# Wendison/FCL-taco2

Hardware: AMD Instinct MI355X
Metric: mel-frames/sec (FCL-taco2-S forward, batch=32, 80-mel) (higher is better)
Workload: dtype f32 via bf16x3-split MFMA operands, fp32 accumulate (max-abs 8e-6 on mel vs the reference; FCL_PRECISION=0 = exact fp32 MFMA)

## Files before the change

### fcl-taco2_amd/csrc/decoder_step.hip

```cpp
#include "fcl_common.h"
#include "lstm_epilogue.h"

namespace fcl {


template <int NT>
__device__ __forceinline__ void rowtile_mma(const float* A_l, int lda_l, const float* const (&wrow)[NT], int K, int r16, int kq,
                                            f32x4 (&out)[NT], int rot = 0) {
    f32x4 acc0[NT], acc1[NT];
#pragma unroll
    for (int t = 0; t < NT; ++t) acc0[t] = acc1[t] = (f32x4){0.f, 0.f, 0.f, 0.f};
    const float* ap = A_l + r16 * lda_l + kq * 4;
    const float* wp[NT];
#pragma unroll
    for (int t = 0; t < NT; ++t) wp[t] = wrow[t] + kq * 4;
    const int nfull = K >> 6;
    f32x4 bn[NT][4];
    int cc = nfull > 0 ? rot % nfull : 0;
    if (nfull > 0) {
#pragma unroll
        for (int t = 0; t < NT; ++t)
#pragma unroll
            for (int i = 0; i < 4; ++i) bn[t][i] = *reinterpret_cast<const f32x4*>(wp[t] + (cc << 6) + i * 16);
    }
    for (int c = 0; c < nfull; ++c) {
        const int k = cc << 6;
        const int cn = cc + 1 == nfull ? 0 : cc + 1;
        f32x4 b[NT][4], a[4];
#pragma unroll
        for (int t = 0; t < NT; ++t)
#pragma unroll
            for (int i = 0; i < 4; ++i) b[t][i] = bn[t][i];
        if (c + 1 < nfull) {
#pragma unroll
            for (int t = 0; t < NT; ++t)
#pragma unroll
                for (int i = 0; i < 4; ++i) bn[t][i] = *reinterpret_cast<const f32x4*>(wp[t] + (cn << 6) + i * 16);
        }
        cc = cn;
#pragma unroll
        for (int i = 0; i < 4; ++i) a[i] = *reinterpret_cast<const f32x4*>(ap + k + i * 16);
        __builtin_amdgcn_sched_barrier(0);
#pragma unroll
        for (int i = 0; i < 4; ++i) {
#pragma unroll
            for (int t = 0; t < NT; ++t) {
                acc0[t] = __builtin_amdgcn_mfma_f32_16x16x4f32(a[i][0], b[t][i][0], acc0[t], 0, 0, 0);
                acc1[t] = __builtin_amdgcn_mfma_f32_16x16x4f32(a[i][1], b[t][i][1], acc1[t], 0, 0, 0);
            }
#pragma unroll
            for (int t = 0; t < NT; ++t) {
                acc0[t] = __builtin_amdgcn_mfma_f32_16x16x4f32(a[i][2], b[t][i][2], acc0[t], 0, 0, 0);
                acc1[t] = __builtin_amdgcn_mfma_f32_16x16x4f32(a[i][3], b[t][i][3], acc1[t], 0, 0, 0);
            }
        }
    }
    for (int k = nfull << 6; k < K; k += 16) {
        const bool in = k + kq * 4 < K;
        f32x4 a = *reinterpret_cast<const f32x4*>(in ? ap + k : A_l + r16 * lda_l);
        if (!in) a = (f32x4){0.f, 0.f, 0.f, 0.f};
#pragma unroll
        for (int t = 0; t < NT; ++t) {
            const f32x4 bb = *reinterpret_cast<const f32x4*>(in ? wp[t] + k : wrow[t]);
            acc0[t] = __builtin_amdgcn_mfma_f32_16x16x4f32(a[0], bb[0], acc0[t], 0, 0, 0);
            acc1[t] = __builtin_amdgcn_mfma_f32_16x16x4f32(a[1], bb[1], acc1[t], 0, 0, 0);
            acc0[t] = __builtin_amdgcn_mfma_f32_16x16x4f32(a[2], bb[2], acc0[t], 0, 0, 0);
            acc1[t] = __builtin_amdgcn_mfma_f32_16x16x4f32(a[3], bb[3], acc1[t], 0, 0, 0);
        }
    }
#pragma unroll
    for (int t = 0; t < NT; ++t) out[t] = acc0[t] + acc1[t];
}

__device__ __forceinline__ void load_rowtile(float* dst, int ld_l, const float* src, int ld, int K, int m0, int M) {
    const int per_row = K >> 2;
    for (int i = threadIdx.x; i < 16 * per_row; i += blockDim.x) {
        const int r = i / per_row, c = (i - r * per_row) * 4;
        const int m = min(m0 + r, M - 1);
        *reinterpret_cast<f32x4*>(dst + r * ld_l + c) = *reinterpret_cast<const f32x4*>(src + (size_t)m * ld + c);
    }
}

__device__ __forceinline__ float drop_apply(float v, int mode, const uint8_t* keep, int ldkeep, int m, int n, int N,
                                            float scale, float p, unsigned int seed) {
    if (mode == 1) return keep[(size_t)m * ldkeep + n] ? v * scale : 0.f;
    if (mode == 2) {
        const unsigned int h = hash_u32(((unsigned int)m * (unsigned int)N + (unsigned int)n) ^ seed);
        return ((h >> 8) * (1.0f / 16777216.0f) >= p) ? v * scale : 0.f;
    }
    return v;
}

__device__ __forceinline__ bool feat_prenet_rows(const FeatPrenetArgs& a, int rows, int& Ms_feat, int& Ms_pre) {
    Ms_feat = (a.live && a.t_prev >= 0) ? min(a.M_feat, a.live[a.t_prev]) : a.M_feat;
    Ms_pre = a.live ? min(a.M_pre, a.live[a.t_cur]) : a.M_pre;
    if (a.live && a.w0 && blockIdx.x == 0 && threadIdx.x == 0 && a.live[a.t_cur] > a.M_pre) atomicOr(a.status, (unsigned int)FCL_STATUS_ROWS_CAP);
    if ((int)blockIdx.x * rows >= (a.h1 ? Ms_feat : Ms_pre)) return false;
    return true;
}

__global__ __launch_bounds__(512) void feat_prenet_kernel(const FeatPrenetArgs a) {
    const int M_feat = a.M_feat, M_pre = a.M_pre;
    int Ms_feat, Ms_pre;
    if (!feat_prenet_rows(a, 16, Ms_feat, Ms_pre)) return;
    extern __shared__ __attribute__((aligned(16))) float smem[];
    const int ldU = a.U + 4, ldO = a.O + 4, ldP = a.P + 4;
    float* A1 = smem;
    float* A2 = A1 + 16 * ldU;
    float* A3 = A2 + 16 * ldO;
    const int m0 = blockIdx.x * 16;
    const int lane = threadIdx.x & 63, wave = threadIdx.x >> 6, nwaves = blockDim.x >> 6;
    const int r16 = lane & 15, kq = lane >> 4;
    const int col = lane & 15, rq = lane >> 4;
    const unsigned int sbump = a.seed_dev ? *a.seed_dev * 0x9E3779B9u : 0u;
    const unsigned int seed0 = hash_u32(a.seed0 + sbump), seed1 = hash_u32(a.seed1 + sbump);

    if (a.h1) {
        load_rowtile(A1, ldU, a.h1, a.U, a.U, m0, M_feat);
        __syncthreads();
        for (int tile = wave; tile * 16 < a.O; tile += nwaves) {
            const float* const wr[1] = {a.wf_h + (size_t)min(tile * 16 + r16, a.O - 1) * a.U};
            const int nc = tile * 16 + col, ncc = min(nc, a.O - 1);
            float f0v[4];
            int fo[4];
#pragma unroll
            for (int r = 0; r < 4; ++r) {
                const int mc = min(m0 + rq * 4 + r, M_feat - 1);
                f0v[r] = a.F0[(size_t)mc * a.O + ncc];
                fo[r] = a.frame_off[mc];
            }
            f32x4 accv[1];
            rowtile_mma<1>(A1, ldU, wr, a.U, r16, kq, accv, blockIdx.x);
            const f32x4 acc = accv[0];
#pragma unroll
            for (int r = 0; r < 4; ++r) {
                const int row = rq * 4 + r, m = m0 + row;
                float v = 0.f;
                if (m < Ms_feat && nc < a.O) {
                    v = acc[r] + f0v[r];
                    a.before[(size_t)(fo[r] + a.t_prev) * a.O + nc] = v;
                }
                if (nc < a.O) A2[row * ldO + nc] = (a.out_act && m < Ms_feat) ? act_apply(v, a.out_act) : v;
            }
        }
    } else {
        for (int i = threadIdx.x; i < 16 * ldO; i += blockDim.x) A2[i] = 0.f;
    }
    if (!a.w0 || m0 >= M_pre) return;
    __syncthreads();
    if (a.teacher_in) {
        load_rowtile(A2, ldO, a.teacher_in, a.teacher_ld, a.O, m0, M_pre);
        __syncthreads();
    }
    for (int tile = wave; tile * 16 < a.P; tile += 2 * nwaves) {
        const int tile2 = tile + nwaves;
        const float* const wr[2] = {a.w0 + (size_t)min(tile * 16 + r16, a.P - 1) * a.O, a.w0 + (size_t)min(tile2 * 16 + r16, a.P - 1) * a.O};
        f32x4 accv[2];
        rowtile_mma<2>(A2, ldO, wr, a.O, r16, kq, accv, blockIdx.x);
#pragma unroll
        for (int tt = 0; tt < 2; ++tt) {
            const int nc = (tt ? tile2 : tile) * 16 + col;
            if (nc < a.P) {
                const float bn = a.b0[nc];
#pragma unroll
                for (int r = 0; r < 4; ++r) {
                    const int row = rq * 4 + r, m = m0 + row;
                    float v = fmaxf(accv[tt][r] + bn, 0.f);
                    if (m < M_pre) v = drop_apply(v, a.drop_mode, a.keep0, a.P, m, nc, a.P, a.keep_scale, a.drop_p, seed0);
                    A3[row * ldP + nc] = v;
                }
            }
        }
    }
    __syncthreads();
    for (int tile = wave; tile * 16 < a.P; tile += 2 * nwaves) {
        const int tile2 = tile + nwaves;
        const float* const wr[2] = {a.w1 + (size_t)min(tile * 16 + r16, a.P - 1) * a.P, a.w1 + (size_t)min(tile2 * 16 + r16, a.P - 1) * a.P};
        f32x4 accv[2];
        rowtile_mma<2>(A3, ldP, wr, a.P, r16, kq, accv, blockIdx.x);
#pragma unroll
        for (int tt = 0; tt < 2; ++tt) {
            const int nc = (tt ? tile2 : tile) * 16 + col;
            if (nc < a.P) {
                const float bn = a.b1[nc];
#pragma unroll
                for (int r = 0; r < 4; ++r) {
                    const int m = m0 + rq * 4 + r;
                    if (m >= Ms_pre) continue;
                    float v = fmaxf(accv[tt][r] + bn, 0.f);
                    v = drop_apply(v, a.drop_mode, a.keep1, a.P, m, nc, a.P, a.keep_scale, a.drop_p, seed1);
                    a.pre_out[(size_t)m * a.P + nc] = v;
                    if (a.tap_prenet) a.tap_prenet[(size_t)(a.frame_off[m] + a.t_cur) * a.P + nc] = v;
                }
            }
        }
    }
}

__device__ __forceinline__ void split1(float x, u16& hi, u16& lo) {
    const __bf16 h = (__bf16)x;
    hi = __builtin_bit_cast(u16, h);
    lo = __builtin_bit_cast(u16, (__bf16)(x - (float)h));
}

template <int NT>
__device__ __forceinline__ void rowtile_mma_x3(const u16* Ah, const u16* Al, int ldk, const u16* const (&fhi)[NT], const u16* const (&flo)[NT],
                                               int K, int r16, int kq, f32x4 (&out)[NT]) {
    f32x4 acc[NT];
#pragma unroll
    for (int t = 0; t < NT; ++t) acc[t] = (f32x4){0.f, 0.f, 0.f, 0.f};
    const u16* ah = Ah + r16 * ldk + kq * 8;
    const u16* al = Al + r16 * ldk + kq * 8;
    const int nsteps = (K + 31) >> 5;
    s16x8 bhn[NT], bln[NT];
#pragma unroll
    for (int t = 0; t < NT; ++t) {
        bhn[t] = *reinterpret_cast<const s16x8*>(fhi[t]);
        bln[t] = *reinterpret_cast<const s16x8*>(flo[t]);
    }
    for (int st = 0; st < nsteps; ++st) {
        const int k = st << 5;
        s16x8 bh[NT], bl[NT];
#pragma unroll
        for (int t = 0; t < NT; ++t) { bh[t] = bhn[t]; bl[t] = bln[t]; }
        if (st + 1 < nsteps) {
#pragma unroll
            for (int t = 0; t < NT; ++t) {
                bhn[t] = *reinterpret_cast<const s16x8*>(fhi[t] + (size_t)(st + 1) * 512);
                bln[t] = *reinterpret_cast<const s16x8*>(flo[t] + (size_t)(st + 1) * 512);
            }
        }
        s16x8 a_hi = {0, 0, 0, 0, 0, 0, 0, 0}, a_lo = {0, 0, 0, 0, 0, 0, 0, 0};
        if (k + kq * 8 < K) {
            a_hi = *reinterpret_cast<const s16x8*>(ah + k);
            a_lo = *reinterpret_cast<const s16x8*>(al + k);
        }
        __builtin_amdgcn_sched_barrier(0);
#pragma unroll
        for (int t = 0; t < NT; ++t) acc[t] = __builtin_amdgcn_mfma_f32_16x16x32_bf16(a_lo, bh[t], acc[t], 0, 0, 0);
#pragma unroll
        for (int t = 0; t < NT; ++t) acc[t] = __builtin_amdgcn_mfma_f32_16x16x32_bf16(a_hi, bl[t], acc[t], 0, 0, 0);
#pragma unroll
        for (int t = 0; t < NT; ++t) acc[t] = __builtin_amdgcn_mfma_f32_16x16x32_bf16(a_hi, bh[t], acc[t], 0, 0, 0);
    }
#pragma unroll
    for (int t = 0; t < NT; ++t) out[t] = acc[t];
}

template <int NT, int NS>
struct WFrag {
    s16x8 hi[NT][NS], lo[NT][NS];
    __device__ __forceinline__ void load(const u16* const (&fhi)[NT], const u16* const (&flo)[NT]) {
#pragma unroll
        for (int t = 0; t < NT; ++t)
#pragma unroll
            for (int st = 0; st < NS; ++st) {
                hi[t][st] = *reinterpret_cast<const s16x8*>(fhi[t] + st * 512);
                lo[t][st] = *reinterpret_cast<const s16x8*>(flo[t] + st * 512);
            }
    }
    __device__ __forceinline__ void mma(const u16* Ah, const u16* Al, int ldk, int K, int r16, int kq, f32x4 (&out)[NT]) const {
        f32x4 acc[NT];
#pragma unroll
        for (int t = 0; t < NT; ++t) acc[t] = (f32x4){0.f, 0.f, 0.f, 0.f};
        const u16* ah = Ah + r16 * ldk + kq * 8;
        const u16* al = Al + r16 * ldk + kq * 8;
#pragma unroll
        for (int st = 0; st < NS; ++st) {
            s16x8 a_hi = {0, 0, 0, 0, 0, 0, 0, 0}, a_lo = {0, 0, 0, 0, 0, 0, 0, 0};
            if (st * 32 + kq * 8 < K) {
                a_hi = *reinterpret_cast<const s16x8*>(ah + st * 32);
                a_lo = *reinterpret_cast<const s16x8*>(al + st * 32);
            }
#pragma unroll
            for (int t = 0; t < NT; ++t) acc[t] = __builtin_amdgcn_mfma_f32_16x16x32_bf16(a_lo, hi[t][st], acc[t], 0, 0, 0);
#pragma unroll
            for (int t = 0; t < NT; ++t) acc[t] = __builtin_amdgcn_mfma_f32_16x16x32_bf16(a_hi, lo[t][st], acc[t], 0, 0, 0);
#pragma unroll
            for (int t = 0; t < NT; ++t) acc[t] = __builtin_amdgcn_mfma_f32_16x16x32_bf16(a_hi, hi[t][st], acc[t], 0, 0, 0);
        }
#pragma unroll
        for (int t = 0; t < NT; ++t) out[t] = acc[t];
    }
};

__device__ __forceinline__ void load_rowtile_split(u16* Ah, u16* Al, int ldk, const float* src, int ld, int K, int m0, int M) {
    const int per_row = K >> 2;
    for (int i = threadIdx.x; i < 16 * per_row; i += blockDim.x) {
        const int r = i / per_row, c = (i - r * per_row) * 4;
        const int m = min(m0 + r, M - 1);
        const f32x4 v = *reinterpret_cast<const f32x4*>(src + (size_t)m * ld + c);
        u16 h[4], l[4];
#pragma unroll
        for (int e = 0; e < 4; ++e) split1(v[e], h[e], l[e]);
        *reinterpret_cast<uint2*>(Ah + r * ldk + c) = make_uint2(h[0] | ((unsigned)h[1] << 16), h[2] | ((unsigned)h[3] << 16));
        *reinterpret_cast<uint2*>(Al + r * ldk + c) = make_uint2(l[0] | ((unsigned)l[1] << 16), l[2] | ((unsigned)l[3] << 16));
    }
}

__global__ __launch_bounds__(512) void feat_prenet_x3_kernel(const FeatPrenetArgs a) {
    const int M_feat = a.M_feat, M_pre = a.M_pre;
    const int Ms_feat = (a.live && a.t_prev >= 0) ? min(a.M_feat, a.live[a.t_prev]) : a.M_feat, Ms_pre = a.live ? min(a.M_pre, a.live[a.t_cur]) : a.M_pre;
    if (a.live && a.w0 && blockIdx.x == 0 && threadIdx.x == 0 && a.live[a.t_cur] > a.M_pre) atomicOr(a.status, (unsigned int)FCL_STATUS_ROWS_CAP);
    if ((int)blockIdx.x * (16) >= (a.h1 ? Ms_feat : Ms_pre)) return;
    extern __shared__ __attribute__((aligned(16))) float smem[];
    const int ldU = a.U + 8, ldO = a.O + 8, ldP = a.P + 8;
    u16* A1h = reinterpret_cast<u16*>(smem);
    u16* A1l = A1h + 16 * ldU;
    u16* A2h = A1l + 16 * ldU;
    u16* A2l = A2h + 16 * ldO;
    u16* A3h = A2l + 16 * ldO;
    u16* A3l = A3h + 16 * ldP;
    const int m0 = blockIdx.x * 16;
    const int lane = threadIdx.x & 63, wave = threadIdx.x >> 6, nwaves = blockDim.x >> 6;
    const int r16 = lane & 15, kq = lane >> 4;
    const int col = lane & 15, rq = lane >> 4;
    const unsigned int sbump = a.seed_dev ? *a.seed_dev * 0x9E3779B9u : 0u;
    const unsigned int seed0 = hash_u32(a.seed0 + sbump), seed1 = hash_u32(a.seed1 + sbump);

    const bool has_pre = a.w0 && m0 < M_pre;
    const int ptile = wave, ptile2 = wave + nwaves;
    const int nsU = (a.U + 31) >> 5, nsO = (a.O + 31) >> 5, nsP = (a.P + 31) >> 5, ptmax = ((a.P + 15) >> 4) - 1;
    const size_t lane8 = (size_t)lane * 8;
    auto frag = [&](const u16* base, int tile, int ns) { return base + (size_t)tile * ns * 512 + lane8; };
    float pb0[2] = {0.f, 0.f}, pb1[2] = {0.f, 0.f};
    if (has_pre) {
#pragma unroll
        for (int tt = 0; tt < 2; ++tt) {
            const int nc = min((tt ? ptile2 : ptile) * 16 + col, a.P - 1);
            pb0[tt] = a.b0[nc];
            pb1[tt] = a.b1[nc];
        }
    }
    if (a.h1) {
        f32x4 accv[1];
        load_rowtile_split(A1h, A1l, ldU, a.h1, a.U, a.U, m0, M_feat);
        __syncthreads();
        if (a.dbg_phase == 1) return;
        for (int tile = wave; tile * 16 < a.O; tile += nwaves) {
            const u16* const wh[1] = {frag(a.wf_hi, tile, nsU)};
            const u16* const wl[1] = {frag(a.wf_lo, tile, nsU)};
            const int nc = tile * 16 + col, ncc = min(nc, a.O - 1);
            float f0v[4];
            int fo[4];
#pragma unroll
            for (int r = 0; r < 4; ++r) {
                const int mc = min(m0 + rq * 4 + r, M_feat - 1);
                f0v[r] = a.F0[(size_t)mc * a.O + ncc];
                fo[r] = a.frame_off[mc];
            }
            rowtile_mma_x3<1>(A1h, A1l, ldU, wh, wl, a.U, r16, kq, accv);
#pragma unroll
            for (int r = 0; r < 4; ++r) {
                const int row = rq * 4 + r, m = m0 + row;
                float v = 0.f;
                if (m < Ms_feat && nc < a.O) {
                    v = accv[0][r] + f0v[r];
                    a.before[(size_t)(fo[r] + a.t_prev) * a.O + nc] = v;
                    if (a.before_p) store_p32(a.before_p, (a.O + 31) >> 5, fo[r] + a.t_prev, nc, v);
                }
                if (nc < a.O) split1((a.out_act && m < Ms_feat) ? act_apply(v, a.out_act) : v, A2h[row * ldO + nc], A2l[row * ldO + nc]);
            }
        }
        if (a.before_p && (a.O & 31)) {
            const int padc = 32 - (a.O & 31);
            for (int i = threadIdx.x; i < 16 * padc; i += blockDim.x) {
                const int m = m0 + i / padc;
                if (m < Ms_feat) store_p32(a.before_p, (a.O + 31) >> 5, a.frame_off[m] + a.t_prev, a.O + i % padc, 0.f);
            }
        }
    } else {
        for (int i = threadIdx.x; i < 16 * ldO; i += blockDim.x) { A2h[i] = 0; A2l[i] = 0; }
    }
    if (!has_pre || a.dbg_phase == 2) return;
    lds_barrier();
    if (a.teacher_in) {
        load_rowtile_split(A2h, A2l, ldO, a.teacher_in, a.teacher_ld, a.O, m0, M_pre);
        __syncthreads();
    }
    for (int tile = wave; tile * 16 < a.P; tile += 2 * nwaves) {
        const int tile2 = tile + nwaves;
        const u16* const wh[2] = {frag(a.w0_hi, tile, nsO), frag(a.w0_hi, min(tile2, ptmax), nsO)};
        const u16* const wl[2] = {frag(a.w0_lo, tile, nsO), frag(a.w0_lo, min(tile2, ptmax), nsO)};
        f32x4 accv[2];
        rowtile_mma_x3<2>(A2h, A2l, ldO, wh, wl, a.O, r16, kq, accv);
#pragma unroll
        for (int tt = 0; tt < 2; ++tt) {
            const int nc = (tt ? tile2 : tile) * 16 + col;
            if (nc < a.P) {
                const float bn = tile == ptile ? pb0[tt] : a.b0[nc];
#pragma unroll
                for (int r = 0; r < 4; ++r) {
                    const int row = rq * 4 + r, m = m0 + row;
                    float v = fmaxf(accv[tt][r] + bn, 0.f);
                    if (m < M_pre) v = drop_apply(v, a.drop_mode, a.keep0, a.P, m, nc, a.P, a.keep_scale, a.drop_p, seed0);
                    split1(v, A3h[row * ldP + nc], A3l[row * ldP + nc]);
                }
            }
        }
    }
    lds_barrier();
    if (a.dbg_phase == 3) return;
    for (int tile = wave; tile * 16 < a.P; tile += 2 * nwaves) {
        const int tile2 = tile + nwaves;
        const u16* const wh[2] = {frag(a.w1_hi, tile, nsP), frag(a.w1_hi, min(tile2, ptmax), nsP)};
        const u16* const wl[2] = {frag(a.w1_lo, tile, nsP), frag(a.w1_lo, min(tile2, ptmax), nsP)};
        f32x4 accv[2];
        rowtile_mma_x3<2>(A3h, A3l, ldP, wh, wl, a.P, r16, kq, accv);
#pragma unroll
        for (int tt = 0; tt < 2; ++tt) {
            const int nc = (tt ? tile2 : tile) * 16 + col;
            if (nc < a.P) {
                const float bn = tile == ptile ? pb1[tt] : a.b1[nc];
#pragma unroll
                for (int r = 0; r < 4; ++r) {
                    const int m = m0 + rq * 4 + r;
                    if (m >= Ms_pre) continue;
                    float v = fmaxf(accv[tt][r] + bn, 0.f);
                    v = drop_apply(v, a.drop_mode, a.keep1, a.P, m, nc, a.P, a.keep_scale, a.drop_p, seed1);
                    if (a.pre_out) a.pre_out[(size_t)m * a.P + nc] = v;
                    if (a.pre_out_p) store_p32(a.pre_out_p, (a.P + 31) >> 5, m, nc, v);
                    if (a.tap_prenet) a.tap_prenet[(size_t)(a.frame_off[m] + a.t_cur) * a.P + nc] = v;
                }
            }
        }
    }
}

__device__ __forceinline__ void p32_store4(unsigned short* __restrict__ p, int ld, long long m, int n, uint2 hi, uint2 lo) {
    unsigned short* line = p + ((size_t)m * ld + (n >> 5)) * 64 + (n & 31);
    *reinterpret_cast<uint2*>(line) = hi;
    *reinterpret_cast<uint2*>(line + 32) = lo;
}

template <int NT, int NS_>
__device__ __forceinline__ void mma_t(const WFrag<NT, NS_>& w, const u16* Ah, const u16* Al, int ldk, int r16, int kq, f32x4 (&out)[NT]) {
    f32x4 acc[NT];
#pragma unroll
    for (int t = 0; t < NT; ++t) acc[t] = (f32x4){0.f, 0.f, 0.f, 0.f};
    const u16* ah = Ah + r16 * ldk + kq * 8;
    const u16* al = Al + r16 * ldk + kq * 8;
#pragma unroll
    for (int st = 0; st < NS_; ++st) {
        const s16x8 a_hi = *reinterpret_cast<const s16x8*>(ah + st * 32);
        const s16x8 a_lo = *reinterpret_cast<const s16x8*>(al + st * 32);
#pragma unroll
        for (int t = 0; t < NT; ++t) acc[t] = __builtin_amdgcn_mfma_f32_16x16x32_bf16(w.hi[t][st], a_lo, acc[t], 0, 0, 0);
#pragma unroll
        for (int t = 0; t < NT; ++t) acc[t] = __builtin_amdgcn_mfma_f32_16x16x32_bf16(w.lo[t][st], a_hi, acc[t], 0, 0, 0);
#pragma unroll
        for (int t = 0; t < NT; ++t) acc[t] = __builtin_amdgcn_mfma_f32_16x16x32_bf16(w.hi[t][st], a_hi, acc[t], 0, 0, 0);
    }
#pragma unroll
    for (int t = 0; t < NT; ++t) out[t] = acc[t];
}

template <int DROP, int RT>
__global__ __launch_bounds__(512) void feat_prenet_split_kernel(const FeatPrenetArgs a) {
    constexpr int SU = 8, SO = 3, SP = 8, U = 256, OP = 96, P = 256;
    const int M_feat = a.M_feat, M_pre = a.M_pre;
    const int Ms_feat = (a.live && a.t_prev >= 0) ? min(a.M_feat, a.live[a.t_prev]) : a.M_feat, Ms_pre = a.live ? min(a.M_pre, a.live[a.t_cur]) : a.M_pre;
    const int split = blockIdx.y;
    if (a.live && a.w0 && blockIdx.x == 0 && split == 0 && threadIdx.x == 0 && a.live[a.t_cur] > a.M_pre) atomicOr(a.status, (unsigned int)FCL_STATUS_ROWS_CAP);
    if ((int)blockIdx.x * (16 * RT) >= (a.h1 ? Ms_feat : Ms_pre)) return;
    constexpr int ldU = U + 16, ldO = OP + 16, ldP = P + 16, ROWS = 16 * RT;
    static_assert(ldU == ldP, "the layer-1 operand tile re-uses the h1 tile's LDS");
    extern __shared__ __attribute__((aligned(16))) u16 fp_lds[];
    u16* A1h = fp_lds;
    u16* A1l = A1h + ROWS * ldU;
    u16* A2h = A1l + ROWS * ldU;
    u16* A2l = A2h + ROWS * ldO;
    u16* A3h = A1h;
    u16* A3l = A1l;
    const int O = a.O;
    const int m0 = blockIdx.x * ROWS;
    const int lane = threadIdx.x & 63, wave = __builtin_amdgcn_readfirstlane(threadIdx.x >> 6);
    const int r16 = lane & 15, kq = lane >> 4;
    const int arow = lane & 15, cq = lane >> 4;
    const bool has_feat = a.h1 != nullptr, has_pre = a.w0 != nullptr && m0 < M_pre;
    if (!has_pre && split != 0) return;
    const bool feat_wave = has_feat && wave * 16 < O;
    const size_t lane8 = (size_t)lane * 8;
    auto frag = [&](const u16* base, int tile, int ns) { return base + (size_t)tile * ns * 512 + lane8; };
    const int t0 = wave, t1 = wave + 8;
    const int c1 = split * 16 + wave * 2;

    constexpr int HV = RT * 2;
    f32x4 hreg[HV];
    if (has_feat) {
#pragma unroll
        for (int j = 0; j < HV; ++j) {
            const int i = threadIdx.x + j * 512, r = i >> 6, c = (i & 63) * 4;
            hreg[j] = *reinterpret_cast<const f32x4*>(a.h1 + (size_t)min(m0 + r, M_feat - 1) * U + c);
        }
    }
    asm volatile("s_barrier" ::: "memory");
    WFrag<1, SU> ff;
    WFrag<2, SO> f0;
    WFrag<2, SP> f1;
    const int fnc = wave * 16 + cq * 4;
    f32x4 f0v[RT];
    int fo[RT];
    if (feat_wave) {
        const u16* const wh[1] = {frag(a.wf_hi, wave, SU)};
        const u16* const wl[1] = {frag(a.wf_lo, wave, SU)};
        ff.load(wh, wl);
    }
#pragma unroll
    for (int q = 0; q < RT; ++q) {
        f0v[q] = (f32x4){0.f, 0.f, 0.f, 0.f};
        fo[q] = 0;
        if (feat_wave && fnc < O) {
            const int mc = min(m0 + q * 16 + arow, M_feat - 1);
            f0v[q] = *reinterpret_cast<const f32x4*>(a.F0 + (size_t)mc * O + fnc);
            if (split == 0) fo[q] = a.frame_off[mc];
        }
    }
    unsigned int seed0 = 0, seed1 = 0;
    const unsigned int thr16 = (unsigned int)(a.drop_p * 65536.0f);
    if (DROP == 2) {
        const unsigned int sbump = a.seed_dev ? *a.seed_dev * 0x9E3779B9u : 0u;
        seed0 = hash_u32(a.seed0 + sbump);
        seed1 = hash_u32(a.seed1 + sbump);
    }
    f32x4 pb0[2], pb1[2];
    unsigned int k0[RT][2], k1[RT][2];
#pragma unroll
    for (int tt = 0; tt < 2; ++tt) pb0[tt] = (f32x4){0.f, 0.f, 0.f, 0.f};
    if (has_feat) asm volatile("s_barrier" ::: "memory");
    if (has_pre) {
        const u16* const wh0[2] = {frag(a.w0_hi, t0, SO), frag(a.w0_hi, t1, SO)};
        const u16* const wl0[2] = {frag(a.w0_lo, t0, SO), frag(a.w0_lo, t1, SO)};
        f0.load(wh0, wl0);
#pragma unroll
        for (int tt = 0; tt < 2; ++tt) {
            const int nc = (tt ? t1 : t0) * 16 + cq * 4;
            pb0[tt] = *reinterpret_cast<const f32x4*>(a.b0 + nc);
            if (DROP == 1) {
#pragma unroll
                for (int q = 0; q < RT; ++q) k0[q][tt] = *reinterpret_cast<const unsigned int*>(a.keep0 + (size_t)min(m0 + q * 16 + arow, M_pre - 1) * P + nc);
            }
        }
    }
    for (int i = threadIdx.x; i < ROWS * ldO / 8; i += 512) {
        reinterpret_cast<uint4*>(A2h)[i] = make_uint4(0, 0, 0, 0);
        reinterpret_cast<uint4*>(A2l)[i] = make_uint4(0, 0, 0, 0);
    }
    if (has_feat) {
#pragma unroll
        for (int j = 0; j < HV; ++j) {
            const int i = threadIdx.x + j * 512, r = i >> 6, c = (i & 63) * 4;
            uint2 h, l;
            split4(hreg[j], h, l);
            *reinterpret_cast<uint2*>(A1h + r * ldU + c) = h;
            *reinterpret_cast<uint2*>(A1l + r * ldU + c) = l;
        }
    }
#pragma unroll
    for (int tt = 0; tt < 2; ++tt) pb1[tt] = (f32x4){0.f, 0.f, 0.f, 0.f};
    auto request_l1 = [&]() {
        if (has_pre) {
            const u16* wh1[2];
            const u16* wl1[2];
#pragma unroll
            for (int tt = 0; tt < 2; ++tt) {
                wh1[tt] = frag(a.w1_hi, c1 + tt, SP);
                wl1[tt] = frag(a.w1_lo, c1 + tt, SP);
            }
            f1.load(wh1, wl1);
#pragma unroll
            for (int tt = 0; tt < 2; ++tt) {
                const int nc = (c1 + tt) * 16 + cq * 4;
                pb1[tt] = *reinterpret_cast<const f32x4*>(a.b1 + nc);
                if (DROP == 1) {
#pragma unroll
                    for (int q = 0; q < RT; ++q) k1[q][tt] = *reinterpret_cast<const unsigned int*>(a.keep1 + (size_t)min(m0 + q * 16 + arow, M_pre - 1) * P + nc);
                }
            }
        }
    };
    lds_barrier();
    if (a.dbg_phase == 1) return;
    if (feat_wave) {
#pragma unroll
        for (int q = 0; q < RT; ++q) {
            f32x4 accv[1];
            mma_t<1, SU>(ff, A1h + q * 16 * ldU, A1l + q * 16 * ldU, ldU, r16, kq, accv);
            const int row = q * 16 + arow, m = m0 + row;
            if (fnc < O) {
                f32x4 v = (f32x4){0.f, 0.f, 0.f, 0.f};
                uint2 h, l;
                if (m < Ms_feat) {
                    v = accv[0] + f0v[q];
                    if (split == 0) {
                        const long long fr = (long long)fo[q] + a.t_prev;
                        *reinterpret_cast<f32x4*>(a.before + (size_t)fr * O + fnc) = v;
                        if (a.before_p) {
                            split4(v, h, l);
                            p32_store4(a.before_p, (O + 31) >> 5, fr, fnc, h, l);
                        }
                    }
                    if (a.out_act) {
#pragma unroll
                        for (int r = 0; r < 4; ++r) v[r] = act_apply(v[r], a.out_act);
                    }
                }
                split4(v, h, l);
                *reinterpret_cast<uint2*>(A2h + row * ldO + fnc) = h;
                *reinterpret_cast<uint2*>(A2l + row * ldO + fnc) = l;
            }
        }
    }
    if (has_feat && split == 0 && a.before_p && (O & 31)) {
        const int padc = 32 - (O & 31);
        for (int i = threadIdx.x; i < ROWS * padc; i += 512) {
            const int m = m0 + i / padc;
            if (m < Ms_feat) store_p32(a.before_p, (O + 31) >> 5, a.frame_off[m] + a.t_prev, O + i % padc, 0.f);
        }
    }
    if (!has_pre || a.dbg_phase == 2) return;
    request_l1();
    lds_barrier();
    if (a.teacher_in) {
#pragma unroll
        for (int q = 0; q < RT; ++q) load_rowtile_split(A2h + q * 16 * ldO, A2l + q * 16 * ldO, ldO, a.teacher_in, a.teacher_ld, O, m0 + q * 16, M_pre);
        lds_barrier();
    }
#pragma unroll
    for (int q = 0; q < RT; ++q) {
        f32x4 accv[2];
        mma_t<2, SO>(f0, A2h + q * 16 * ldO, A2l + q * 16 * ldO, ldO, r16, kq, accv);
        const int row = q * 16 + arow, m = m0 + row;
#pragma unroll
        for (int tt = 0; tt < 2; ++tt) {
            const int nc = (tt ? t1 : t0) * 16 + cq * 4;
            f32x4 v = accv[tt] + pb0[tt];
#pragma unroll
            for (int r = 0; r < 4; ++r) v[r] = fmaxf(v[r], 0.f);
            v = drop4<DROP>(v, DROP == 1 ? k0[q][tt] : 0u, (unsigned int)m * (unsigned int)P + (unsigned int)nc, seed0, thr16, a.keep_scale);
            uint2 h, l;
            split4(v, h, l);
            *reinterpret_cast<uint2*>(A3h + row * ldP + nc) = h;
            *reinterpret_cast<uint2*>(A3l + row * ldP + nc) = l;
        }
    }
    lds_barrier();
    if (a.dbg_phase == 3) return;
#pragma unroll
    for (int q = 0; q < RT; ++q) {
        f32x4 accv[2];
        mma_t<2, SP>(f1, A3h + q * 16 * ldP, A3l + q * 16 * ldP, ldP, r16, kq, accv);
        const int m = m0 + q * 16 + arow;
        if (m >= Ms_pre) continue;
#pragma unroll
        for (int tt = 0; tt < 2; ++tt) {
            const int nc = (c1 + tt) * 16 + cq * 4;
            f32x4 v = accv[tt] + pb1[tt];
#pragma unroll
            for (int r = 0; r < 4; ++r) v[r] = fmaxf(v[r], 0.f);
            v = drop4<DROP>(v, DROP == 1 ? k1[q][tt] : 0u, (unsigned int)m * (unsigned int)P + (unsigned int)nc, seed1, thr16, a.keep_scale);
            if (a.pre_out) *reinterpret_cast<f32x4*>(a.pre_out + (size_t)m * P + nc) = v;
            if (a.pre_out_p) {
                uint2 h, l;
                split4(v, h, l);
                p32_store4(a.pre_out_p, SP, m, nc, h, l);
            }
            if (a.tap_prenet) *reinterpret_cast<f32x4*>(a.tap_prenet + (size_t)(a.frame_off[m] + a.t_cur) * P + nc) = v;
        }
    }
}


template <int NT, int NS_>
struct WFragF {
    f32x4 w0[NT][NS_], w1[NT][NS_];
    __device__ __forceinline__ void load(const float* const (&f)[NT]) {
#pragma unroll
        for (int t = 0; t < NT; ++t)
#pragma unroll
            for (int st = 0; st < NS_; ++st) {
                w0[t][st] = *reinterpret_cast<const f32x4*>(f[t] + st * 512);
                w1[t][st] = *reinterpret_cast<const f32x4*>(f[t] + st * 512 + 4);
            }
    }
};

template <int NT, int NS_>
__device__ __forceinline__ void mma_tf(const WFragF<NT, NS_>& w, const float* A, int ldk, int r16, int kq, f32x4 (&out)[NT]) {
    f32x4 acc[NT];
#pragma unroll
    for (int t = 0; t < NT; ++t) acc[t] = (f32x4){0.f, 0.f, 0.f, 0.f};
    const float* a = A + r16 * ldk + kq * 4;
#pragma unroll
    for (int st = 0; st < NS_; ++st) {
        const f32x4 a0 = *reinterpret_cast<const f32x4*>(a + st * 32), a1 = *reinterpret_cast<const f32x4*>(a + st * 32 + 16);
#pragma unroll
        for (int e = 0; e < 4; ++e)
#pragma unroll
            for (int t = 0; t < NT; ++t) acc[t] = __builtin_amdgcn_mfma_f32_16x16x4f32(w.w0[t][st][e], a0[e], acc[t], 0, 0, 0);
#pragma unroll
        for (int e = 0; e < 4; ++e)
#pragma unroll
            for (int t = 0; t < NT; ++t) acc[t] = __builtin_amdgcn_mfma_f32_16x16x4f32(w.w1[t][st][e], a1[e], acc[t], 0, 0, 0);
    }
#pragma unroll
    for (int t = 0; t < NT; ++t) out[t] = acc[t];
}

template <int DROP>
__global__ __launch_bounds__(512) void feat_prenet_split_f32_kernel(const FeatPrenetArgs a) {
    constexpr int SU = 8, SO = 3, SP = 8, U = 256, OP = 96, P = 256;
    const int M_feat = a.M_feat, M_pre = a.M_pre;
    int Ms_feat, Ms_pre;
    if (!feat_prenet_rows(a, 16, Ms_feat, Ms_pre)) return;
    constexpr int ldU = U + 8, ldO = OP + 8, ldP = P + 8;
    static_assert(ldU == ldP, "the layer-1 operand tile re-uses the h1 tile's LDS");
    extern __shared__ __attribute__((aligned(16))) float fpf_lds[];
    float* A1 = fpf_lds;
    float* A2 = A1 + 16 * ldU;
    const int O = a.O;
    const int m0 = blockIdx.x * 16;
    const int lane = threadIdx.x & 63, wave = __builtin_amdgcn_readfirstlane(threadIdx.x >> 6);
    const int r16 = lane & 15, kq = lane >> 4;
    const int arow = lane & 15, cq = lane >> 4;
    const bool has_feat = a.h1 != nullptr, has_pre = a.w0 != nullptr && m0 < M_pre;
    const bool feat_wave = has_feat && wave * 16 < O;
    const size_t lane8 = (size_t)lane * 8;
    auto frag = [&](const float* base, int tile, int ns) { return base + (size_t)tile * ns * 512 + lane8; };
    const int t0 = wave, t1 = wave + 8;
    f32x4 hreg[2];
    if (has_feat) {
#pragma unroll
        for (int j = 0; j < 2; ++j) {
            const int i = threadIdx.x + j * 512, r = i >> 6, c = (i & 63) * 4;
            hreg[j] = *reinterpret_cast<const f32x4*>(a.h1 + (size_t)min(m0 + r, M_feat - 1) * U + c);
        }
    }
    asm volatile("s_barrier" ::: "memory");
    WFragF<1, SU> ff;
    WFragF<2, SO> f0;
    WFragF<2, SP> f1;
    const int fnc = wave * 16 + cq * 4;
    f32x4 f0v = (f32x4){0.f, 0.f, 0.f, 0.f};
    int fo = 0;
    if (feat_wave) {
        const float* const wf[1] = {frag(a.wf_ff, wave, SU)};
        ff.load(wf);
        if (fnc < O) {
            const int mc = min(m0 + arow, M_feat - 1);
            f0v = *reinterpret_cast<const f32x4*>(a.F0 + (size_t)mc * O + fnc);
            fo = a.frame_off[mc];
        }
    }
    unsigned int seed0 = 0, seed1 = 0;
    const unsigned int thr16 = (unsigned int)(a.drop_p * 65536.0f);
    if (DROP == 2) {
        const unsigned int sbump = a.seed_dev ? *a.seed_dev * 0x9E3779B9u : 0u;
        seed0 = hash_u32(a.seed0 + sbump);
        seed1 = hash_u32(a.seed1 + sbump);
    }
    f32x4 pb0[2], pb1[2];
    unsigned int k0[2] = {0u, 0u}, k1[2] = {0u, 0u};
#pragma unroll
    for (int tt = 0; tt < 2; ++tt) pb0[tt] = pb1[tt] = (f32x4){0.f, 0.f, 0.f, 0.f};
    if (has_feat) asm volatile("s_barrier" ::: "memory");
    if (has_pre) {
        const float* const w0p[2] = {frag(a.w0_ff, t0, SO), frag(a.w0_ff, t1, SO)};
        f0.load(w0p);
#pragma unroll
        for (int tt = 0; tt < 2; ++tt) {
            const int nc = (tt ? t1 : t0) * 16 + cq * 4;
            pb0[tt] = *reinterpret_cast<const f32x4*>(a.b0 + nc);
            if (DROP == 1) k0[tt] = *reinterpret_cast<const unsigned int*>(a.keep0 + (size_t)min(m0 + arow, M_pre - 1) * P + nc);
        }
    }
    for (int i = threadIdx.x; i < 16 * ldO / 4; i += 512) reinterpret_cast<f32x4*>(A2)[i] = (f32x4){0.f, 0.f, 0.f, 0.f};
    if (has_feat) {
#pragma unroll
        for (int j = 0; j < 2; ++j) {
            const int i = threadIdx.x + j * 512, r = i >> 6, c = (i & 63) * 4;
            *reinterpret_cast<f32x4*>(A1 + r * ldU + c) = hreg[j];
        }
    }
    lds_barrier();
    if (feat_wave) {
        f32x4 accv[1];
        mma_tf<1, SU>(ff, A1, ldU, r16, kq, accv);
        const int m = m0 + arow;
        if (fnc < O) {
            f32x4 v = (f32x4){0.f, 0.f, 0.f, 0.f};
            if (m < Ms_feat) {
                v = accv[0] + f0v;
                *reinterpret_cast<f32x4*>(a.before + (size_t)((long long)fo + a.t_prev) * O + fnc) = v;
                if (a.out_act) {
#pragma unroll
                    for (int r = 0; r < 4; ++r) v[r] = act_apply(v[r], a.out_act);
                }
            }
            *reinterpret_cast<f32x4*>(A2 + arow * ldO + fnc) = v;
        }
    }
    if (!has_pre) return;
    {
        const float* const w1p[2] = {frag(a.w1_ff, t0, SP), frag(a.w1_ff, t1, SP)};
        f1.load(w1p);
#pragma unroll
        for (int tt = 0; tt < 2; ++tt) {
            const int nc = (tt ? t1 : t0) * 16 + cq * 4;
            pb1[tt] = *reinterpret_cast<const f32x4*>(a.b1 + nc);
            if (DROP == 1) k1[tt] = *reinterpret_cast<const unsigned int*>(a.keep1 + (size_t)min(m0 + arow, M_pre - 1) * P + nc);
        }
    }
    lds_barrier();
    {
        f32x4 accv[2];
        mma_tf<2, SO>(f0, A2, ldO, r16, kq, accv);
        const int m = m0 + arow;
#pragma unroll
        for (int tt = 0; tt < 2; ++tt) {
            const int nc = (tt ? t1 : t0) * 16 + cq * 4;
            f32x4 v = accv[tt] + pb0[tt];
#pragma unroll
            for (int r = 0; r < 4; ++r) v[r] = fmaxf(v[r], 0.f);
            v = drop4<DROP>(v, k0[tt], (unsigned int)m * (unsigned int)P + (unsigned int)nc, seed0, thr16, a.keep_scale);
            *reinterpret_cast<f32x4*>(A1 + arow * ldP + nc) = v;
        }
    }
    lds_barrier();
    {
        f32x4 accv[2];
        mma_tf<2, SP>(f1, A1, ldP, r16, kq, accv);
        const int m = m0 + arow;
        if (m >= Ms_pre) return;
#pragma unroll
        for (int tt = 0; tt < 2; ++tt) {
            const int nc = (tt ? t1 : t0) * 16 + cq * 4;
            f32x4 v = accv[tt] + pb1[tt];
#pragma unroll
            for (int r = 0; r < 4; ++r) v[r] = fmaxf(v[r], 0.f);
            v = drop4<DROP>(v, k1[tt], (unsigned int)m * (unsigned int)P + (unsigned int)nc, seed1, thr16, a.keep_scale);
            if (a.pre_out) *reinterpret_cast<f32x4*>(a.pre_out + (size_t)m * P + nc) = v;
            if (a.tap_prenet) *reinterpret_cast<f32x4*>(a.tap_prenet + (size_t)(a.frame_off[m] + a.t_cur) * P + nc) = v;
        }
    }
}

__device__ __forceinline__ void gates_to_cell(const LstmStepArgs& a, int g, int lane, const f32x4& acc, bool units_in_lane, int m, int u, bool valid, int Ms,
                                              const CellIn& ci) {
    __shared__ float g_l[4][16][17];
    const int lo = lane & 15, hi = lane >> 4;
#pragma unroll
    for (int i = 0; i < 4; ++i) {
        if (units_in_lane) g_l[g][lo][hi * 4 + i] = acc[i];
        else g_l[g][hi * 4 + i][lo] = acc[i];
    }
    __syncthreads();
    if (!valid || m >= Ms) return;
    const int row = threadIdx.x >> 4, uc = threadIdx.x & 15;
    const float pre[4] = {g_l[0][row][uc], g_l[1][row][uc], g_l[2][row][uc], g_l[3][row][uc]};
    cell_finish(a, m, u, pre, ci);
}

template <bool PRE>
__global__ __launch_bounds__(256) void lstm_small_x3_kernel(const LstmStepArgs a) {
    const int M = a.M, Ms = live_rows_of(a.M, a.m_dev);
    if ((int)blockIdx.y * 16 >= Ms) return;
    constexpr int KC = 512;
    __shared__ __attribute__((aligned(16))) u16 A_h[16 * (KC + 16)];
    __shared__ __attribute__((aligned(16))) u16 A_lo[16 * (KC + 16)];
    const int m0 = blockIdx.y * 16, u0 = blockIdx.x * 16;
    const int lane = threadIdx.x & 63, g = threadIdx.x >> 6;
    const int r16 = lane & 15, kq = lane >> 4;
    const int erow = threadIdx.x >> 4, euc = threadIdx.x & 15;
    const int em = m0 + erow, eu = u0 + euc;
    const bool evalid = em < M && eu < a.U;
    CellIn ci;
    if (evalid) ci = cell_prefetch(a, em, eu);
    f32x4 acc = {0.f, 0.f, 0.f, 0.f};
    WFrag<1, 8> wf[2];
    if (PRE) {
        const int nt = a.nterms;
#pragma unroll
        for (int t = 0; t < 2; ++t) {
            if (t >= nt) break;
            const size_t fo = (size_t)((g * a.U + u0) >> 4) * 8 * 512 + (size_t)lane * 8;
            const u16* const wh[1] = {a.term[t].Whi + fo};
            const u16* const wl[1] = {a.term[t].Wlo + fo};
            wf[t].load(wh, wl);
        }
#pragma unroll
        for (int t = 0; t < 2; ++t) {
            if (t >= nt) break;
            if (t) __syncthreads();
            load_rowtile_split(A_h, A_lo, 256 + 16, a.term[t].A, a.term[t].lda, 256, m0, M);
            __syncthreads();
            f32x4 part[1];
            wf[t].mma(A_h, A_lo, 256 + 16, 256, r16, kq, part);
            acc += part[0];
        }
    }
    for (int t = 0; t < (PRE ? 0 : a.nterms); ++t) {
        const GemmTerm T = a.term[t];
        for (int k0 = 0; k0 < T.K; k0 += KC) {
            const int kc = min(KC, T.K - k0);
            __syncthreads();
            load_rowtile_split(A_h, A_lo, kc + 16, T.A + k0, T.lda, kc, m0, M);
            __syncthreads();
            const size_t fo = ((size_t)((g * a.U + u0) >> 4) * ((T.K + 31) >> 5) + (k0 >> 5)) * 512 + (size_t)lane * 8;
            const u16* const wh[1] = {T.Whi + fo};
            const u16* const wl[1] = {T.Wlo + fo};
            f32x4 part[1];
            rowtile_mma_x3<1>(A_h, A_lo, kc + 16, wh, wl, kc, r16, kq, part);
            acc += part[0];
        }
    }
    gates_to_cell(a, g, lane, acc, false, em, eu, evalid, Ms, ci);
}


__global__ __launch_bounds__(256) void lstm_small_ff_kernel(const LstmStepArgs a) {
    const int M = a.M, Ms = live_rows_of(a.M, a.m_dev);
    if ((int)blockIdx.y * 16 >= Ms) return;
    constexpr int LD = 256 + 8;
    __shared__ __attribute__((aligned(16))) float A_f[16 * LD];
    const int m0 = blockIdx.y * 16, u0 = blockIdx.x * 16;
    const int lane = threadIdx.x & 63, g = threadIdx.x >> 6;
    const int r16 = lane & 15, kq = lane >> 4;
    const int erow = threadIdx.x >> 4, euc = threadIdx.x & 15;
    const int em = m0 + erow, eu = u0 + euc;
    const bool evalid = em < M && eu < a.U;
    CellIn ci;
    if (evalid) ci = cell_prefetch(a, em, eu);
    f32x4 acc = {0.f, 0.f, 0.f, 0.f};
    WFragF<1, 8> wf[2];
    const int nt = a.nterms;
#pragma unroll
    for (int t = 0; t < 2; ++t) {
        if (t >= nt) break;
        const float* const w[1] = {a.term[t].Wff + (size_t)((g * a.U + u0) >> 4) * 8 * 512 + (size_t)lane * 8};
        wf[t].load(w);
    }
#pragma unroll
    for (int t = 0; t < 2; ++t) {
        if (t >= nt) break;
        if (t) __syncthreads();
        load_rowtile(A_f, LD, a.term[t].A, a.term[t].lda, 256, m0, M);
        __syncthreads();
        f32x4 part[1];
        mma_tf<1, 8>(wf[t], A_f, LD, r16, kq, part);
        acc += part[0];
    }
    gates_to_cell(a, g, lane, acc, true, em, eu, evalid, Ms, ci);
}

constexpr int SMALL_KC = 512;

__device__ __forceinline__ void lstm_small_body(const LstmStepArgs& a) {
    const int M = a.M, Ms = live_rows_of(a.M, a.m_dev);
    if ((int)blockIdx.y * 16 >= Ms) return;
    __shared__ __attribute__((aligned(16))) float A_l[16 * (SMALL_KC + 4)];
    __shared__ float g_l[4][16][17];
    const int m0 = blockIdx.y * 16, u0 = blockIdx.x * 16;
    const int lane = threadIdx.x & 63, g = threadIdx.x >> 6;
    const int r16 = lane & 15, kq = lane >> 4;
    const int u = u0 + r16;
    f32x4 acc = {0.f, 0.f, 0.f, 0.f};
    for (int t = 0; t < a.nterms; ++t) {
        const GemmTerm T = a.term[t];
        for (int k0 = 0; k0 < T.K; k0 += SMALL_KC) {
            const int kc = min(SMALL_KC, T.K - k0);
            __syncthreads();
            load_rowtile(A_l, kc + 4, T.A + k0, T.lda, kc, m0, M);
            __syncthreads();
            const float* const wr[1] = {T.W + (size_t)(g * a.U + min(u, a.U - 1)) * T.ldw + k0};
            f32x4 part[1];
            rowtile_mma<1>(A_l, kc + 4, wr, kc, r16, kq, part, blockIdx.y);
            acc += part[0];
        }
    }
    {
        const int col = lane & 15, rq = lane >> 4;
#pragma unroll
        for (int r = 0; r < 4; ++r) g_l[g][rq * 4 + r][col] = acc[r];
    }
    __syncthreads();
    const int row = threadIdx.x >> 4, uc = threadIdx.x & 15;
    const int m = m0 + row, uu = u0 + uc;
    if (m >= Ms || uu >= a.U) return;
    const CellIn ci = cell_prefetch(a, m, uu);
    const float pre[4] = {g_l[0][row][uc], g_l[1][row][uc], g_l[2][row][uc], g_l[3][row][uc]};
    cell_finish(a, m, uu, pre, ci);
}

__global__ __launch_bounds__(256) void lstm_small_kernel(const LstmStepArgs a) { lstm_small_body(a); }

__global__ __launch_bounds__(256) void lstm_small_pair_kernel(const LstmStepArgs a0, const LstmStepArgs a1) {
    if (blockIdx.z == 0) lstm_small_body(a0);
    else lstm_small_body(a1);
}

int launch_lstm_small(const LstmStepArgs& a, hipStream_t s) {
    const double fl = lstm_step_flops(a);
    dim3 grid((a.U + 15) / 16, (a.M + 15) / 16);
    bool planes = true;
    for (int i = 0; i < a.nterms; ++i) planes = planes && a.term[i].Whi && a.term[i].Wlo && (a.term[i].K & 7) == 0 && a.term[i].ldw == a.term[i].K;
    planes = planes && (a.U & 15) == 0;
    bool pre256 = a.nterms == 2 || (a.nterms == 1 && !a.h_in), ff = true;
    for (int i = 0; i < a.nterms; ++i) {
        pre256 = pre256 && a.term[i].K == 256;
        ff = ff && a.term[i].Wff != nullptr;
    }
    if (planes) {
        ProfScope ps("lstm_small_kernel/bf16x3", fl, a.M, s);
        if (pre256) hipLaunchKernelGGL(lstm_small_x3_kernel<true>, grid, dim3(256), 0, s, a);
        else hipLaunchKernelGGL(lstm_small_x3_kernel<false>, grid, dim3(256), 0, s, a);
    } else if (pre256 && ff && (a.U & 15) == 0) {
        ProfScope ps("lstm_small_ff_kernel/f32", fl, a.M, s);
        hipLaunchKernelGGL(lstm_small_ff_kernel, grid, dim3(256), 0, s, a);
    } else {
        ProfScope ps("lstm_small_kernel", fl, a.M, s);
        hipLaunchKernelGGL(lstm_small_kernel, grid, dim3(256), 0, s, a);
    }
    return check_hip(hipGetLastError(), "lstm_small launch");
}

int launch_lstm_small_pair(const LstmStepArgs& a0, const LstmStepArgs& a1, hipStream_t s) {
    const double fl = lstm_step_flops(a0) + lstm_step_flops(a1);
    const int mmax = a0.M > a1.M ? a0.M : a1.M;
    dim3 grid((a0.U + 15) / 16, (mmax + 15) / 16, 2);
    ProfScope ps("lstm_small_pair_kernel", fl, a0.M + a1.M, s);
    hipLaunchKernelGGL(lstm_small_pair_kernel, grid, dim3(256), 0, s, a0, a1);
    return check_hip(hipGetLastError(), "lstm_small_pair launch");
}

int launch_lstm_small_pair_any(const LstmStepArgs& a0, const LstmStepArgs& a1, hipStream_t s, bool* handled) {
    *handled = false;
    if (a0.U != a1.U || a0.m_dev || a1.m_dev) return 0;
    for (const LstmStepArgs* a : {&a0, &a1})
        for (int i = 0; i < a->nterms; ++i)
            if (!a->term[i].A || !a->term[i].W || a->term[i].Whi || a->term[i].Wff) return 0;
    *handled = true;
    return launch_lstm_small_pair(a0, a1, s);
}

static int launch_fp_drop(const void* const (&fn)[3], int drop_mode, dim3 grid, size_t lds, const FeatPrenetArgs& a, hipStream_t s) {
    const void* f = fn[drop_mode == 1 || drop_mode == 2 ? drop_mode : 0];
    const int rc = ensure_dyn_lds(f, (int)lds);
    if (rc) return rc;
    void* args[] = {const_cast<FeatPrenetArgs*>(&a)};
    return check_hip(hipLaunchKernel(f, grid, dim3(512), args, lds, s), "feat_prenet launch");
}

template <int RT>
static int launch_feat_prenet_split(const FeatPrenetArgs& a, int rows, hipStream_t s) {
    constexpr size_t lds_s = 2 * sizeof(unsigned short) * 16 * RT * ((256 + 16) + (96 + 16));
    static const void* const fn[3] = {reinterpret_cast<const void*>(feat_prenet_split_kernel<0, RT>), reinterpret_cast<const void*>(feat_prenet_split_kernel<1, RT>),
                                      reinterpret_cast<const void*>(feat_prenet_split_kernel<2, RT>)};
    return launch_fp_drop(fn, a.drop_mode, dim3((rows + 16 * RT - 1) / (16 * RT), 1), lds_s, a, s);
}

int launch_feat_prenet(const FeatPrenetArgs& a, hipStream_t s) {
    const int rows = a.h1 ? a.M_feat : a.M_pre;
    if (rows <= 0) return 0;
    FCL_REQUIRE(!(a.U & 3) && !(a.O & 3) && !(a.P & 3), FCL_ERR_SHAPE, "feat_prenet: U/O/P must be multiples of 4");
    const size_t lds = sizeof(float) * 16 * ((size_t)(a.U + 4) + (a.O + 4) + (a.P + 4));
    FCL_REQUIRE(lds <= 160 * 1024, FCL_ERR_SHAPE, "feat_prenet: tile does not fit LDS (%zu B)", lds);
    {
        const int rc = ensure_dyn_lds(reinterpret_cast<const void*>(feat_prenet_kernel), 160 * 1024);
        if (rc) return rc;
    }
    double fl = 0;
    if (a.h1) fl += 2.0 * a.M_feat * a.O * a.U;
    if (a.w0) fl += 2.0 * a.M_pre * ((double)a.P * a.O + (double)a.P * a.P);
    static const int dbg = tunable("FP_DBG", 0);
    const_cast<FeatPrenetArgs&>(a).dbg_phase = dbg;
    const bool planes = a.wf_hi && a.wf_lo && a.w0_hi && a.w0_lo && a.w1_hi && a.w1_lo && !(a.U & 7) && !(a.O & 7) && !(a.P & 7);
    FCL_REQUIRE(planes || (!a.pre_out_p && !a.before_p), FCL_ERR_INVALID, "feat_prenet: P32 outputs need the bf16x3 weight planes");
    FCL_REQUIRE(!a.w0 || a.pre_out || a.pre_out_p, FCL_ERR_INVALID, "feat_prenet: no prenet output buffer");
    FCL_REQUIRE(!a.pre_out_p || !(a.P & 31), FCL_ERR_SHAPE, "feat_prenet: P32 prenet output needs P %% 32 == 0");
    if (planes) {
        const size_t lds3 = 2 * sizeof(unsigned short) * 16 * ((size_t)(a.U + 8) + (a.O + 8) + (a.P + 8));
        {
            const int rc = ensure_dyn_lds(reinterpret_cast<const void*>(feat_prenet_x3_kernel), 160 * 1024);
            if (rc) return rc;
        }
        ProfScope ps("feat_prenet_kernel/bf16x3", fl, rows, s);
        if (a.U == 256 && a.O > 64 && a.O <= 96 && a.P == 256) {
            const int rc = rows >= 4096 ? launch_feat_prenet_split<2>(a, rows, s) : launch_feat_prenet_split<1>(a, rows, s);
            if (rc) return rc;
        } else {
            hipLaunchKernelGGL(feat_prenet_x3_kernel, dim3((rows + 15) / 16), dim3(512), lds3, s, a);
        }
    } else if (a.wf_ff && a.w0_ff && a.w1_ff && a.U == 256 && a.P == 256 && a.O > 64 && a.O <= 96 && !a.teacher_in && !a.pre_out_p && !a.before_p &&
               (!a.w0 || a.pre_out)) {
        ProfScope ps("feat_prenet_split_kernel/f32", fl, rows, s);
        constexpr size_t lds_f = sizeof(float) * 16 * ((256 + 8) + (96 + 8));
        static const void* const fn[3] = {reinterpret_cast<const void*>(feat_prenet_split_f32_kernel<0>), reinterpret_cast<const void*>(feat_prenet_split_f32_kernel<1>),
                                          reinterpret_cast<const void*>(feat_prenet_split_f32_kernel<2>)};
        const int rc = launch_fp_drop(fn, a.drop_mode, dim3((rows + 15) / 16), lds_f, a, s);
        if (rc) return rc;
    } else {
        ProfScope ps("feat_prenet_kernel", fl, rows, s);
        hipLaunchKernelGGL(feat_prenet_kernel, dim3((rows + 15) / 16), dim3(512), lds, s, a);
    }
    return check_hip(hipGetLastError(), "feat_prenet launch");
}

}
```

Baseline: 49.29 million.

## Stage both small-LSTM input tiles at once and overlap weight loads with staging

The small LSTM step kernels (x3 and ff) used to stage and multiply the two GEMM terms one after another, with barriers between them. They now issue the activation row loads for both terms into registers first, then load the weight fragments in two halves around the LDS store. Both terms sit side by side in a wider LDS tile, so a single __syncthreads replaces the per-term barrier pairs. This is meant to hide global-memory latency in these latency-bound per-step kernels, at the cost of more live registers and a larger shared-memory tile for the ff kernel.

```diff
diff --git a/fcl-taco2_amd/csrc/decoder_step.hip b/fcl-taco2_amd/csrc/decoder_step.hip
--- a/fcl-taco2_amd/csrc/decoder_step.hip
+++ b/fcl-taco2_amd/csrc/decoder_step.hip
@@ -250,11 +250,12 @@
 template <int NT, int NS>
 struct WFrag {
     s16x8 hi[NT][NS], lo[NT][NS];
+    template <int S0 = 0, int S1 = NS>
     __device__ __forceinline__ void load(const u16* const (&fhi)[NT], const u16* const (&flo)[NT]) {
 #pragma unroll
         for (int t = 0; t < NT; ++t)
 #pragma unroll
-            for (int st = 0; st < NS; ++st) {
+            for (int st = S0; st < S1; ++st) {
                 hi[t][st] = *reinterpret_cast<const s16x8*>(fhi[t] + st * 512);
                 lo[t][st] = *reinterpret_cast<const s16x8*>(flo[t] + st * 512);
             }
@@ -674,11 +675,12 @@
 template <int NT, int NS_>
 struct WFragF {
     f32x4 w0[NT][NS_], w1[NT][NS_];
+    template <int S0 = 0, int S1 = NS_>
     __device__ __forceinline__ void load(const float* const (&f)[NT]) {
 #pragma unroll
         for (int t = 0; t < NT; ++t)
 #pragma unroll
-            for (int st = 0; st < NS_; ++st) {
+            for (int st = S0; st < S1; ++st) {
                 w0[t][st] = *reinterpret_cast<const f32x4*>(f[t] + st * 512);
                 w1[t][st] = *reinterpret_cast<const f32x4*>(f[t] + st * 512 + 4);
             }
@@ -861,6 +863,97 @@
     cell_finish(a, m, u, pre, ci);
 }
 
+struct RowTile256 {
+    f32x4 v[4];
+    __device__ __forceinline__ void request(const float* src, int ld, int m0, int M) {
+#pragma unroll
+        for (int j = 0; j < 4; ++j) {
+            const int i = threadIdx.x + j * 256, r = i >> 6, c = (i & 63) * 4;
+            v[j] = *reinterpret_cast<const f32x4*>(src + (size_t)min(m0 + r, M - 1) * ld + c);
+        }
+    }
+    __device__ __forceinline__ void split_store(u16* Ah, u16* Al, int ldk) const {
+#pragma unroll
+        for (int j = 0; j < 4; ++j) {
+            const int i = threadIdx.x + j * 256, r = i >> 6, c = (i & 63) * 4;
+            u16 h[4], l[4];
+#pragma unroll
+            for (int e = 0; e < 4; ++e) split1(v[j][e], h[e], l[e]);
+            *reinterpret_cast<uint2*>(Ah + r * ldk + c) = make_uint2(h[0] | ((unsigned)h[1] << 16), h[2] | ((unsigned)h[3] << 16));
+            *reinterpret_cast<uint2*>(Al + r * ldk + c) = make_uint2(l[0] | ((unsigned)l[1] << 16), l[2] | ((unsigned)l[3] << 16));
+        }
+    }
+    __device__ __forceinline__ void store(float* dst, int ld_l) const {
+#pragma unroll
+        for (int j = 0; j < 4; ++j) {
+            const int i = threadIdx.x + j * 256, r = i >> 6, c = (i & 63) * 4;
+            *reinterpret_cast<f32x4*>(dst + r * ld_l + c) = v[j];
+        }
+    }
+};
+
+constexpr int kSmallStepsAtEntry = 4;
+
+template <int NT>
+__device__ __forceinline__ f32x4 small_x3_walk(const LstmStepArgs& a, u16* A_h, u16* A_lo, int ldk, int m0, int M, int g, int u0, int lane) {
+    const int r16 = lane & 15, kq = lane >> 4;
+    RowTile256 rows[NT];
+#pragma unroll
+    for (int t = 0; t < NT; ++t) rows[t].request(a.term[t].A, a.term[t].lda, m0, M);
+    asm volatile("s_barrier" ::: "memory");
+    const size_t fo = (size_t)((g * a.U + u0) >> 4) * 8 * 512 + (size_t)lane * 8;
+    WFrag<1, 8> wf[NT];
+    const u16* const wh0[1] = {a.term[0].Whi + fo};
+    const u16* const wl0[1] = {a.term[0].Wlo + fo};
+    const u16* const wh1[1] = {a.term[NT - 1].Whi + fo};
+    const u16* const wl1[1] = {a.term[NT - 1].Wlo + fo};
+    wf[0].load(wh0, wl0);
+    if (NT > 1) wf[NT - 1].template load<0, kSmallStepsAtEntry>(wh1, wl1);
+    __builtin_amdgcn_sched_barrier(0);
+#pragma unroll
+    for (int t = 0; t < NT; ++t) rows[t].split_store(A_h + t * 256, A_lo + t * 256, ldk);
+    asm volatile("" ::: "memory");
+    if (NT > 1) wf[NT - 1].template load<kSmallStepsAtEntry, 8>(wh1, wl1);
+    __syncthreads();
+    f32x4 acc = {0.f, 0.f, 0.f, 0.f};
+#pragma unroll
+    for (int t = 0; t < NT; ++t) {
+        f32x4 part[1];
+        wf[t].mma(A_h + t * 256, A_lo + t * 256, ldk, 256, r16, kq, part);
+        acc += part[0];
+    }
+    return acc;
+}
+
+template <int NT>
+__device__ __forceinline__ f32x4 small_ff_walk(const LstmStepArgs& a, float* A_f, int ld, int m0, int M, int g, int u0, int lane) {
+    const int r16 = lane & 15, kq = lane >> 4;
+    RowTile256 rows[NT];
+#pragma unroll
+    for (int t = 0; t < NT; ++t) rows[t].request(a.term[t].A, a.term[t].lda, m0, M);
+    asm volatile("s_barrier" ::: "memory");
+    const size_t fo = (size_t)((g * a.U + u0) >> 4) * 8 * 512 + (size_t)lane * 8;
+    WFragF<1, 8> wf[NT];
+    const float* const w0[1] = {a.term[0].Wff + fo};
+    const float* const w1[1] = {a.term[NT - 1].Wff + fo};
+    wf[0].load(w0);
+    if (NT > 1) wf[NT - 1].template load<0, kSmallStepsAtEntry>(w1);
+    __builtin_amdgcn_sched_barrier(0);
+#pragma unroll
+    for (int t = 0; t < NT; ++t) rows[t].store(A_f + t * 256, ld);
+    asm volatile("" ::: "memory");
+    if (NT > 1) wf[NT - 1].template load<kSmallStepsAtEntry, 8>(w1);
+    __syncthreads();
+    f32x4 acc = {0.f, 0.f, 0.f, 0.f};
+#pragma unroll
+    for (int t = 0; t < NT; ++t) {
+        f32x4 part[1];
+        mma_tf<1, 8>(wf[t], A_f + t * 256, ld, r16, kq, part);
+        acc += part[0];
+    }
+    return acc;
+}
+
 template <bool PRE>
 __global__ __launch_bounds__(256) void lstm_small_x3_kernel(const LstmStepArgs a) {
     const int M = a.M, Ms = live_rows_of(a.M, a.m_dev);
@@ -877,28 +970,7 @@
     CellIn ci;
     if (evalid) ci = cell_prefetch(a, em, eu);
     f32x4 acc = {0.f, 0.f, 0.f, 0.f};
-    WFrag<1, 8> wf[2];
-    if (PRE) {
-        const int nt = a.nterms;
-#pragma unroll
-        for (int t = 0; t < 2; ++t) {
-            if (t >= nt) break;
-            const size_t fo = (size_t)((g * a.U + u0) >> 4) * 8 * 512 + (size_t)lane * 8;
-            const u16* const wh[1] = {a.term[t].Whi + fo};
-            const u16* const wl[1] = {a.term[t].Wlo + fo};
-            wf[t].load(wh, wl);
-        }
-#pragma unroll
-        for (int t = 0; t < 2; ++t) {
-            if (t >= nt) break;
-            if (t) __syncthreads();
-            load_rowtile_split(A_h, A_lo, 256 + 16, a.term[t].A, a.term[t].lda, 256, m0, M);
-            __syncthreads();
-            f32x4 part[1];
-            wf[t].mma(A_h, A_lo, 256 + 16, 256, r16, kq, part);
-            acc += part[0];
-        }
-    }
+    if (PRE) acc = a.nterms == 2 ? small_x3_walk<2>(a, A_h, A_lo, KC + 16, m0, M, g, u0, lane) : small_x3_walk<1>(a, A_h, A_lo, KC + 16, m0, M, g, u0, lane);
     for (int t = 0; t < (PRE ? 0 : a.nterms); ++t) {
         const GemmTerm T = a.term[t];
         for (int k0 = 0; k0 < T.K; k0 += KC) {
@@ -921,35 +993,17 @@
 __global__ __launch_bounds__(256) void lstm_small_ff_kernel(const LstmStepArgs a) {
     const int M = a.M, Ms = live_rows_of(a.M, a.m_dev);
     if ((int)blockIdx.y * 16 >= Ms) return;
-    constexpr int LD = 256 + 8;
+    constexpr int LD = 512 + 8;
     __shared__ __attribute__((aligned(16))) float A_f[16 * LD];
     const int m0 = blockIdx.y * 16, u0 = blockIdx.x * 16;
     const int lane = threadIdx.x & 63, g = threadIdx.x >> 6;
-    const int r16 = lane & 15, kq = lane >> 4;
     const int erow = threadIdx.x >> 4, euc = threadIdx.x & 15;
     const int em = m0 + erow, eu = u0 + euc;
     const bool evalid = em < M && eu < a.U;
     CellIn ci;
     if (evalid) ci = cell_prefetch(a, em, eu);
     f32x4 acc = {0.f, 0.f, 0.f, 0.f};
-    WFragF<1, 8> wf[2];
-    const int nt = a.nterms;
-#pragma unroll
-    for (int t = 0; t < 2; ++t) {
-        if (t >= nt) break;
-        const float* const w[1] = {a.term[t].Wff + (size_t)((g * a.U + u0) >> 4) * 8 * 512 + (size_t)lane * 8};
-        wf[t].load(w);
-    }
-#pragma unroll
-    for (int t = 0; t < 2; ++t) {
-        if (t >= nt) break;
-        if (t) __syncthreads();
-        load_rowtile(A_f, LD, a.term[t].A, a.term[t].lda, 256, m0, M);
-        __syncthreads();
-        f32x4 part[1];
-        mma_tf<1, 8>(wf[t], A_f, LD, r16, kq, part);
-        acc += part[0];
-    }
+    acc = a.nterms == 2 ? small_ff_walk<2>(a, A_f, LD, m0, M, g, u0, lane) : small_ff_walk<1>(a, A_f, LD, m0, M, g, u0, lane);
     gates_to_cell(a, g, lane, acc, true, em, eu, evalid, Ms, ci);
 }
 
```

New measurement: 50.62 million, median of 6. 2.7% higher.
